# umr-lops/xsarsea

Hardware: AMD Instinct MI355X
Metric: Mpixels/s wind inversion (CMOD5.N, 20k x 20k sigma0) (higher is better)
Workload: dtype f64; 1 GPU; CMOD5.N mono-VV inversion (the metric's raster), 20000x20000 float32 sigma0/incidence + complex64 ancillary, default LUT 501x499x181 (90319 candidates/pixel), complex64 out, algo=pruned, sigma0 -> dB fused on the device; lines=20000, samples=20000, lines_rank0=20000, parallelism=row tiles x1

## Files before the change

xsarsea_amd/csrc/xsw_band.hpp:

```cpp
#pragma once
#include "xsw_device.hpp"

namespace xsw {

#ifndef XSW_BAND_MAX
#define XSW_BAND_MAX 64
#endif
#ifndef XSW_BAND_RAY_D
#define XSW_BAND_RAY_D 2
#endif
#ifndef XSW_LONG_RUN_MAX
#define XSW_LONG_RUN_MAX 128
#endif
#ifndef XSW_LONG_RUN_MAX_CUT
#define XSW_LONG_RUN_MAX_CUT 64
#endif
#ifndef XSW_SWEEP_MAX
#define XSW_SWEEP_MAX 128
#endif
#ifndef XSW_TAIL_SWEEP
#define XSW_TAIL_SWEEP 256
#endif
#ifndef XSW_B2_HARD_AREA
#define XSW_B2_HARD_AREA 256
#endif
#ifndef XSW_BAND_SEEDED
#define XSW_BAND_SEEDED 1
#endif
#ifndef XSW_BAND_RAYS
#define XSW_BAND_RAYS 3
#endif
#ifndef XSW_BAND_WG_WAVES
#define XSW_BAND_WG_WAVES 4
#endif
#ifndef XSW_BAND_WAVES
#define XSW_BAND_WAVES 8
#endif
#ifndef XSW_BAND_BATCH_S
#define XSW_BAND_BATCH_S 2
#endif
#ifndef XSW_BAND_BATCH
#define XSW_BAND_BATCH 4
#endif
#ifndef XSW_BAND_WAVES_CR
#define XSW_BAND_WAVES_CR 7
#endif
#ifndef XSW_BAND2_WAVES
#define XSW_BAND2_WAVES 4
#endif

struct BandSlot {
    double sn, thr_lo, thr_hi, ah, bh, m2;
    int inc_bin , rows , ipn ;
    int bin_hi ;
};

struct BandRec {
    double s, ah, bh;
    float d;
    int inc_tail;
    int rows;
    int ipn;
    unsigned idx;
    int flags;
};
struct Band2Slot;
constexpr int kBand2SlotBytes = 56;
template <typename T, typename TO, bool CR>
__device__ __forceinline__ void band2_core(const DevTables &L, const KArgs &A, const BandRec &r, bool in, bool searchable, int lane, Band2Slot *__restrict__ slots,
                                           int *__restrict__ res_, long long strip);

__device__ __forceinline__ unsigned long long ballot64(bool b) { return __builtin_amdgcn_ballot_w64(b); }

#ifndef XSW_BOUND_SLACK
#define XSW_BOUND_SLACK 4e-6f
#endif
#ifndef XSW_ARC_G
#define XSW_ARC_G 8
#endif
__device__ __forceinline__ unsigned window_arc(const unsigned short *__restrict__ inv_rows, const float *__restrict__ csphi32, int phi_pad, float wh0, float whs,
                                               bool on, int i_inc, int bin, int bhi, float uhx, float uhy, float jub, int ip_lo, int ncols, int w_lo, int w_hi)
{
    constexpr int G = XSW_ARC_G;
    static_assert(G == 4 || G == 8, "directions per table read");
    const int ii = on ? i_inc : 0;
    const unsigned short *__restrict__ inv_a = inv_rows + mul24_sv((unsigned)phi_pad, (unsigned)(ii * XSW_INV_BINS + (on ? bin : 0)));
    const unsigned short *__restrict__ inv_b = inv_rows + mul24_sv((unsigned)phi_pad, (unsigned)(ii * XSW_INV_BINS + (on ? min(bhi, XSW_INV_BINS - 1) : 0)));
    const bool capped = bhi < XSW_INV_BINS;
    const float m2 = uhx * uhx + uhy * uhy;
    int first = 0x7fff, last = -1;
    const int g0 = on ? (ip_lo & ~(G - 1)) : 0, ip_end = on ? ip_lo + ncols : 0;
    const int ngroups = wave_max_i(on ? (ip_end - g0 + G - 1) / G : 0);
#pragma unroll 1
    for (int k = 0; k < ngroups; ++k) {
        const int gp = g0 + k * G;
        const bool gact = on && gp < ip_end;
        const int gc = gact ? gp : 0;
        unsigned wa[G / 2], wb[G / 2];
        if constexpr (G == 8) {
            const uint4 qa = *(const uint4 *)(inv_a + gc), qb = *(const uint4 *)(inv_b + gc);
            wa[0] = qa.x; wa[1] = qa.y; wa[2] = qa.z; wa[3] = qa.w; wb[0] = qb.x; wb[1] = qb.y; wb[2] = qb.z; wb[3] = qb.w;
        } else {
            const uint2 qa = *(const uint2 *)(inv_a + gc), qb = *(const uint2 *)(inv_b + gc);
            wa[0] = qa.x; wa[1] = qa.y; wb[0] = qb.x; wb[1] = qb.y;
        }
#pragma unroll
        for (int h = 0; h < G / 2; ++h) {
            const float4 c4 = ((const float4 *)((const float2 *)csphi32 + gc))[h];
#pragma unroll
            for (int e = 0; e < 2; ++e) {
                const int ip = gc + 2 * h + e;
                const int ra = (int)((wa[h] >> (e * 16)) & 0xffffu), rb = (int)((wb[h] >> (e * 16)) & 0xffffu);
                const float uh = e ? uhx * c4.z + uhy * c4.w : uhx * c4.x + uhy * c4.y;
                const int lo = max(w_lo, ra), hi = capped ? min(w_hi, rb - 1) : w_hi;
                const float t = vminf(vmaxf(uh, fmaf((float)lo, whs, wh0)), fmaf((float)max(hi, lo), whs, wh0));
                const float jw = fmaf(t, t - 2.0f * uh, m2) - XSW_BOUND_SLACK * (m2 + t * (t + 2.0f * fabsf(uh)));
                const bool live = gact && ip >= ip_lo && ip < ip_end && lo <= hi && !(jw > jub);
                first = (live && first == 0x7fff) ? ip : first;
                last = live ? ip : last;
            }
        }
    }
    return last >= 0 ? (unsigned)first | ((unsigned)last << 16) : 0x00007fffu;
}
__device__ __forceinline__ double ld_co(const char *__restrict__ base, unsigned off0, int row, unsigned rowB)
{
    return *(const double *)(base + (off0 + __umul24((unsigned)row, rowB)));
}

#ifndef XSW_CHORD_MRG
#define XSW_CHORD_MRG 2e-3
#endif
template <int S, int K, bool COUNT>
__device__ __forceinline__ void co_band_pass(const DevTables &L, double inv_dsig, int lane,
                                             const BandSlot *slots , int *res ,
                                             int first, int count , unsigned &cand)
{
    constexpr int sweep_max = XSW_BAND_MAX;
    const double inf = __builtin_inf();
    const int q = lane / S, sl = lane & (S - 1);
    const bool valid = q < count;
    const int owner = valid ? first + q : lane;
    BandSlot B = slots[owner];
    if (!valid) { B.inc_bin = 0; B.rows = 0; B.ipn = 0; B.bin_hi = -1; }
    const int B_ip_lo = B.ipn & 0xffff, B_ncols = (int)((unsigned)B.ipn >> 16);
    const int w_lo = B.rows & 0xffff, w_hi = B.rows >> 16;
    const double thr_lo = B.thr_lo, thr_hi = B.thr_hi, sn = B.sn;
    const double wh0 = 0.5 * L.w0, whs = L.wstep_half;
    const char *__restrict__ base = (const char *)L.co;
    const unsigned rowB = (unsigned)L.phi_pad * 8u;
    const int i_inc = B.inc_bin & 0xffff;
    const unsigned slice0 = mul24_sv(rowB, mul24_sv((unsigned)L.n_w, (unsigned)i_inc));
    const unsigned short *__restrict__ inv_tab = L.inv_rows;
    const unsigned inv_rowB = (unsigned)L.phi_pad * 2u;
    const unsigned inv0 = mul24_sv(inv_rowB, (unsigned)(i_inc * XSW_INV_BINS) + ((unsigned)B.inc_bin >> 16));
    const unsigned inv1 = mul24_sv(inv_rowB, (unsigned)(i_inc * XSW_INV_BINS) + (unsigned)max(B.bin_hi, 0));
    double best = inf, second = inf;
    int brow = 0, bip = 0;
    unsigned ncand = 0;
    bool overflow = false;
    const int nchunks = S == 64 ? (__builtin_amdgcn_readfirstlane(B_ncols) + 64 * K - 1) / (64 * K) : 1;
#pragma unroll 1
    for (int ch = 0; ch < nchunks; ++ch) {
        bool act[K];
        int ip[K], r[K], nrow[K];
        unsigned off0[K];
        double U[K];
#pragma unroll
        for (int j = 0; j < K; ++j) {
            const int vcol = sl + S * j + S * K * ch;
            act[j] = valid && vcol < B_ncols;
            ip[j] = B_ip_lo + (act[j] ? vcol : 0);
            const unsigned ipB = (unsigned)ip[j] * 8u;
            const double2 cs = *(const double2 *)((const char *)L.csphi + 2u * ipB);
            U[j] = 2.0 * (B.ah * cs.x + B.bh * cs.y);
            off0[j] = slice0 + ipB;
        }
        int nmax = 0;
#pragma unroll
        for (int j = 0; j < K; ++j) {
            const unsigned o_first = inv0 + (unsigned)ip[j] * 2u, o_last = inv1 + (unsigned)ip[j] * 2u;
            const int ra = (int)*(const unsigned short *)((const char *)inv_tab + o_first);
            const int rb = (int)*(const unsigned short *)((const char *)inv_tab + o_last);
            r[j] = max(ra, w_lo);
            const int last = B.bin_hi >= 0 ? min(rb - 1, w_hi) : w_hi;
            nrow[j] = act[j] ? last - r[j] + 1 : 0;
            nmax = max(nmax, nrow[j]);
        }
#pragma unroll 1
        for (int t = 0; t < XSW_BAND_MAX; ++t) {
            unsigned long long left[K], any_left = 0ULL;
#pragma unroll
            for (int j = 0; j < K; ++j) { left[j] = ballot64(t < nrow[j]); any_left |= left[j]; }
            if (any_left == 0ULL) break;
#pragma unroll
            for (int j = 0; j < K; ++j) {
                if (left[j] == 0ULL) continue;
                const int rc = min(r[j] + t, w_hi);
                const double v = ld_co(base, off0[j], rc, rowB);
                const bool inb = t < nrow[j];
                const double wh = fma((double)rc, whs, wh0);
                const double dd = fma(v, inv_dsig, sn);
                double J = fma(dd, dd, wh * (wh - U[j]));
                J = __hiloint2double(inb ? __double2hiint(J) : 0x7FE00000, __double2loint(J));
                second = vmin(second, vmax(J, best));
                const bool lt = J < best;
                brow = lt ? rc : brow;
                if (K > 1 || S == 64) bip = lt ? ip[j] : bip;
                best = vmin(best, J);
                if (COUNT) ncand += inb ? 1u : 0u;
            }
        }
        const bool any = nmax > sweep_max;
        overflow = overflow || any;
        if (K == 1 && S != 64) bip = ip[0];
    }
    const int bflat = (int)__umul24((unsigned)brow, (unsigned)L.n_phi) + bip;
    const double gmin = S == 64 ? wave_min_d(best) : seg_min_d<S>(best);
    const double T = gmin + 1e-9 * (1.0 + fabs(gmin) + slots[owner].m2);
    const unsigned long long amb = ballot64(valid && (second <= T || overflow)), surv = ballot64(valid && best <= T);
    const unsigned long long segmask = S == 64 ? ~0ULL : (((1ULL << (S & 63)) - 1ULL) << ((q * S) & 63));
    const bool bad = (amb & segmask) != 0ULL || __popcll(surv & segmask) != 1 || !(gmin < 1e300);
    if (valid && ((!bad && best <= T) || (bad && sl == 0))) res[owner] = bad ? -1 : bflat;
    if (COUNT) {
        unsigned c = ncand;
        for (int off = 32; off > 0; off >>= 1) c += __shfl_xor(c, off);
        cand += c;
    }
}

__device__ __forceinline__ bool list_append(unsigned *__restrict__ count, unsigned *__restrict__ list, unsigned cap, bool flag, long long i, int lane)
{
    const unsigned long long um = __ballot(flag);
    if (!um) return false;
    unsigned base = 0;
    if (lane == 0) base = atomicAdd(count, (unsigned)__popcll(um));
    base = (unsigned)__builtin_amdgcn_readfirstlane((int)base);
    const unsigned at = base + __builtin_amdgcn_mbcnt_hi((unsigned)(um >> 32), __builtin_amdgcn_mbcnt_lo((unsigned)um, 0u));
    if (flag && at < cap) list[at] = (unsigned)i;
    return flag && at >= cap;
}
__device__ __forceinline__ void mask_mark(unsigned long long *__restrict__ mask, bool flag, long long i, long long strip, long long samples, int lane)
{
    const unsigned long long m = __ballot(flag);
    if (!m) return;
    if (strip >= 0) {
        if (lane == 0) atomicOr(&mask[strip], m);
    } else if (flag) {
        const long long ln = i / samples, sm = i - ln * samples;
        atomicOr(&mask[ln * ((samples + 63) >> 6) + (sm >> 6)], 1ULL << (sm & 63));
    }
}

template <typename T, typename TO, bool CR, bool COUNT>
__device__ __forceinline__ void wave_tail(const DevTables &L, const KArgs &A, long long i, bool in, int lane, int flags, int my_flat, long long strip,
                                          unsigned cand, int chain_slot = 0 )
{
    const bool to_b = A.list_b != nullptr && (flags & F_TO_B) != 0, to_c = (flags & F_TO_C) != 0;
    const double nan = __builtin_nan("");
    int my_icr = -1;
    const bool need_co = (flags & F_NEED_CO) != 0;
    bool unresolved = in && need_co && my_flat < 0;

    bool need_cr = false;
    if (CR && A.s_cr) {
        const double inc = ld<T>(A.inc, i);
        const T x = ((const T *)A.s_cr)[i];
        const double s_cr = to_db(x, A.is_db);
        const double dsig = A.dsig_cr ? (double)((const T *)A.dsig_cr)[i] : (double)(T)(x * (T)0 + (T)A.dsig_cr_scalar);
        need_cr = in && !(flags & (F_EARLY_NAN | F_CR_RAW_NAN)) && s_cr == s_cr && dsig == dsig;
        const bool here = need_cr && !unresolved;
        const int i_inc_cr = here ? nearest_index(L.inc_cr, L.n_inc_cr, inc, L.inc_cr_uniform != 0, L.inc_cr0, L.inv_inccrstep) : 0;
        const double aco = (here && need_co) ? L.abs_co[my_flat] : nan;
        bool undecided = here;
        const bool done = L.inv_cr ? search_cr_scan(L, here, i_inc_cr, s_cr, dsig, need_co, aco, my_icr, undecided)
                                   : search_cr_interval(L, here, i_inc_cr, s_cr, dsig, need_co, aco, my_icr, undecided);
        unresolved = unresolved || (need_cr && (undecided || !done));
        if (need_cr) flags |= F_NEED_CR;
    }
    if (COUNT && A.stats) {
        const unsigned long long done_co = __ballot(in && need_co && my_flat >= 0), done_cr = __ballot(need_cr && !unresolved);
        if (lane == 0) {
            atomicAdd(&A.stats[0], (unsigned long long)__popcll(done_co));
            atomicAdd(&A.stats[1], (unsigned long long)cand);
            if (chain_slot && A.stats_chain) atomicAdd(&A.stats[chain_slot], (unsigned long long)cand);
            atomicAdd(&A.stats[3], (unsigned long long)__popcll(done_cr));
        }
    }
    bool drop_b = false, drop_c = false;
    if (A.list_b) drop_b = A.rec_b ? (unresolved && to_b) : list_append(A.list_b_count, A.list_b, A.list_b_cap, unresolved && to_b, i, lane);
    if (A.list_c) drop_c = list_append(A.list_c_count, A.list_c, A.list_c_cap, unresolved && to_c && !to_b, i, lane);
    const bool for_c = A.list_c != nullptr && to_c && !to_b && !drop_c;
    const bool drop_g = list_append(A.list_count, A.list, A.list_cap, unresolved && !to_b && !for_c, i, lane);
    if (A.mask_g) {
        if (A.list_b) mask_mark(A.mask_b, drop_b, i, strip, A.samples, lane);
        mask_mark(A.mask_g, drop_g, i, strip, A.samples, lane);
    }
    if (in) {
        if (!unresolved) {
            Pixel Q;
            Q.flags = flags;
            Q.a_re = nan; Q.a_im = nan;
            if (A.anc) {
                typename Cx<T>::type z = ((const typename Cx<T>::type *)A.anc)[i];
                Q.a_re = (double)z.x;
                Q.a_im = (double)z.y;
            }
            store_pixel<TO, CR>(L, A, i, Q, my_flat, my_icr);
        }
    }
}

template <typename T, typename TO, bool CR, bool COUNT, int ROLE = 0>
__device__ __forceinline__ void band_wave(const DevTables &L, const KArgs &A, long long i, bool in, int lane, BandSlot *__restrict__ slots,
                                          int *__restrict__ res_, bool strip_walk = false ,
                                          long long strip = -1 )
{
    const double nan = __builtin_nan("");
    int flags, my_flat = -1, my_icr = -1;
    unsigned cand = 0;
    constexpr int NC = 11;
    int pos = -1, first[NC] = {}, ncls[NC] = {};
    bool skip = false;
    {
        Pixel P;
        load_pixel<T, false>(L, A, i, in, P);
        flags = P.flags;
        if (CR && A.s_cr) {
            const T x = ((const T *)A.s_cr)[i];
            const T dr = A.dsig_cr ? ((const T *)A.dsig_cr)[i] : (T)0;
            if (x != x || dr != dr) flags |= F_CR_RAW_NAN;
        }
        const unsigned long long todo = __ballot((P.flags & F_NEED_CO) != 0);
        bool eligb = false;
        int ncols_p = 0;
        if (todo) {
            bool loose = false;
            CoWindow W = co_window_lanes<XSW_BAND_RAYS, XSW_BAND_RAY_D, XSW_BAND_SEEDED != 0>(L, P, A.inv_dsig_co, fabs(A.dsig_co), loose);
            int w_hi_e = W.w_hi;
            bool has_tail = false;
            if (L.tail_min) {
                const bool fin1 = (P.flags & F_NEED_CO) != 0 && (P.flags & F_CO_FINITE) != 0;
                const int mono1 = L.mono_rows[fin1 ? P.i_inc : 0];
                if (fin1 && W.w_hi >= mono1 && W.ip_hi >= W.ip_lo) {
                    const int len = W.ip_hi - W.ip_lo + 1, k = min(31 - __clz(len), XSW_TAIL_LEVELS);
                    const double *tk = L.tail_min + mul24_sv((unsigned)L.phi_pad, (unsigned)(P.i_inc * (XSW_TAIL_LEVELS + 1) + k));
                    const double lo = fmin(tk[W.ip_lo], tk[k < XSW_TAIL_LEVELS ? W.ip_hi - (1 << k) + 1 : W.ip_lo]);
                    if (P.s_co + W.band_d < lo) w_hi_e = mono1 - 1;
                    else if (ROLE != 0 && mono1 >= 1 && W.w_hi - mono1 + 1 <= A.tail_max) { has_tail = true; w_hi_e = mono1 - 1; }
                }
            }
            const int nrows_p = w_hi_e - W.w_lo + 1;
            ncols_p = W.ip_hi - W.ip_lo + 1;
            const bool need = (P.flags & F_NEED_CO) != 0 && (P.flags & F_CO_FINITE) != 0 && ncols_p >= 1 && (nrows_p >= 1 || has_tail);
            if (ROLE == 2 && strip_walk) skip = !need || !(w_hi_e < L.mono_rows[need ? P.i_inc : 0]);
            eligb = need && w_hi_e < L.mono_rows[need ? P.i_inc : 0];
            if (ROLE != 2 && need && !eligb) flags |= F_TO_C;
            if (COUNT) cand += (unsigned)__popcll(__ballot(eligb)) * (unsigned)(2 * (32 - __clz((L.n_w + 1) >> 1)) + (XSW_BAND_RAYS - 1) * 2 * XSW_RAY_SIDE_STEPS);
            double thr_lo = P.s_co - W.band_d, thr_hi = P.s_co + W.band_d;
            int bin = 0, bhi = XSW_INV_BINS;
            if (eligb) {
                const double *g = L.inv_grid + 3 * P.i_inc;
                const double t0 = g[0], width = g[1];
                bin = (int)fmin(fmax((thr_lo - t0) * g[2], 0.0), (double)(XSW_INV_BINS - 1));
                if (bin > 0 && fma((double)bin, width, t0) > thr_lo) --bin;
                if (bin > 0 && fma((double)bin, width, t0) > thr_lo) bin = 0;
                bhi = (int)fmin(fmax((thr_hi - t0) * g[2], -1.0), (double)XSW_INV_BINS) + 1;
                if (bhi < XSW_INV_BINS && !(fma((double)bhi, width, t0) > thr_hi)) ++bhi;
                if (bhi < XSW_INV_BINS && !(fma((double)bhi, width, t0) > thr_hi)) bhi = XSW_INV_BINS;
            }
            if (ROLE != 0 && A.arc_min < 0x7fffffff) {
                const bool widep = eligb && !has_tail && ncols_p >= A.arc_min;
                if (__popcll(__ballot(widep)) >= A.arc_crowd) {
                    const double rs = W.band_d * fabs(A.inv_dsig_co);
                    const float jub32 = (float)(rs * rs) * (1.0f + 1e-5f) + 1e-5f;
                    double *park;
                    if constexpr (ROLE == 2) park = (double *)((char *)slots + lane * kBand2SlotBytes);
                    else park = (double *)&slots[lane];
                    park[0] = thr_lo; park[1] = thr_hi; park[2] = W.band_d; park[3] = P.s_co;
                    __asm__ volatile("" ::: "memory");
                    const unsigned arc = window_arc(L.inv_rows, (const float *)L.csphi32, L.phi_pad, (float)(0.5 * L.w0), (float)L.wstep_half, widep, P.i_inc, bin, bhi,
                                                    (float)(0.5 * P.a_re), (float)(0.5 * P.b_eff), jub32, W.ip_lo, ncols_p, W.w_lo, w_hi_e);
                    __asm__ volatile("" ::: "memory");
                    thr_lo = park[0]; thr_hi = park[1]; W.band_d = park[2]; P.s_co = park[3];
                    const int a_first = (int)(arc & 0xffffu), a_last = (int)(arc >> 16);
                    if (widep && a_last >= a_first) {
                        W.ip_lo = a_first;
                        ncols_p = a_last - a_first + 1;
                    }
                }
            }
            bool hard = false;
            int myc = NC;
            if (eligb) {
                const int nv = ncols_p;
                const int p2 = 31 - __clz(max(nv, 2) - 1);
                myc = nv <= 4 ? 0 : min(2 * p2 - 3 + (nv > (3 << (p2 - 1)) ? 1 : 0), NC - 1);
            }
            if (ROLE == 1 || (ROLE == 2 && strip_walk)) {
                int run = 0;
                if (eligb) {
                    const unsigned tab0 = (unsigned)(P.i_inc * XSW_INV_BINS);
                    auto run_at = [&](int ip) {
                        const int ra = (int)L.inv_rows[mul24_sv((unsigned)L.phi_pad, tab0 + (unsigned)bin) + (unsigned)ip];
                        const int rb = bhi < XSW_INV_BINS ? (int)L.inv_rows[mul24_sv((unsigned)L.phi_pad, tab0 + (unsigned)bhi) + (unsigned)ip] : w_hi_e + 1;
                        return min(rb - 1, w_hi_e) - max(ra, W.w_lo) + 1;
                    };
                    run = run_at(P.ipr);
                    if (has_tail) run = max(run, 0) + (W.w_hi - w_hi_e);
                }
                const bool long_one = eligb && run > ((w_hi_e < W.w_hi && !has_tail) ? XSW_LONG_RUN_MAX_CUT : XSW_LONG_RUN_MAX);
                const bool big_area = eligb && !long_one && run * ncols_p > A.area_max;
                const bool crowded = __popcll(__ballot(big_area)) >= A.b2_crowd;
                if (big_area && crowded && run * ncols_p <= A.area_crowd_max) flags |= F_B2_CROWD;
                if (long_one || (big_area && (flags & F_B2_CROWD) == 0)) {
                    myc = NC;
                    eligb = false;
                    if (ROLE == 2) skip = true;
                    if (ROLE == 1) flags |= F_TO_C;
                }
                hard = has_tail || run * ncols_p >= XSW_B2_HARD_AREA || ncols_p >= 64;
                const bool handed = eligb && (run >= A.long_run || has_tail || ncols_p >= A.wide_min);
                if (ROLE == 1 && handed) {
                    myc = NC;
                    eligb = false;
                    flags |= F_TO_B;
                }
                if (ROLE == 2 && eligb && !handed) {
                    myc = NC;
                    eligb = false;
                    skip = true;
                }
            }
            int base = 0;
#pragma unroll
            for (int c = 0; c < NC; ++c) {
                const unsigned long long m = __ballot(myc == c);
                const int rank = (int)__builtin_amdgcn_mbcnt_hi((unsigned)(m >> 32), __builtin_amdgcn_mbcnt_lo((unsigned)m, 0u));
                pos = myc == c ? base + rank : pos;
                first[c] = base;
                ncls[c] = __popcll(m);
                base += ncls[c];
            }
#pragma unroll
            for (int c = 0; c + 1 < NC; ++c) {
                const int np = 64 / (2 << (c >> 1)), npn = 64 / (2 << ((c + 1) >> 1));
                const int rem = ncls[c] % np;
                const int added = (ncls[c + 1] + rem + npn - 1) / npn - (ncls[c + 1] + npn - 1) / npn;
                if (rem > 0 && added == 0) { ncls[c] -= rem; ncls[c + 1] += rem; first[c + 1] -= rem; }
            }
#pragma unroll
            for (int c = 0; c < NC; ++c) {
                first[c] = __builtin_amdgcn_readfirstlane(first[c]);
                ncls[c] = __builtin_amdgcn_readfirstlane(ncls[c]);
            }
            const bool to_rec = ROLE == 1 && A.rec_b != nullptr && (flags & F_TO_B) != 0;
            if constexpr (ROLE == 2) {
                const bool mine = in && !(strip_walk && (skip || (flags & F_NEED_CO) == 0));
                BandRec r;
                r.s = P.s_co; r.ah = 0.5 * P.a_re; r.bh = 0.5 * P.b_eff; r.d = __double2float_ru(W.band_d);
                r.inc_tail = P.i_inc | ((has_tail ? W.w_hi - w_hi_e : 0) << 16);
                r.rows = W.w_lo | (w_hi_e << 16); r.ipn = W.ip_lo | (ncols_p << 16);
                r.idx = (unsigned)i; r.flags = flags | F_B2_HARD;
                band2_core<T, TO, CR>(L, A, r, mine, mine && eligb, lane, (Band2Slot *)slots, res_, strip);
                return;
            }
            BandSlot b;
            if (eligb) {
                const double ah = 0.5 * P.a_re, bh = 0.5 * P.b_eff;
                b.sn = -P.s_co * A.inv_dsig_co; b.thr_lo = thr_lo; b.thr_hi = thr_hi;
                b.ah = ah; b.bh = bh; b.m2 = ah * ah + bh * bh;
                b.inc_bin = P.i_inc | (bin << 16); b.rows = W.w_lo | (w_hi_e << 16); b.ipn = W.ip_lo | (ncols_p << 16);
                b.bin_hi = bhi < XSW_INV_BINS ? bhi : -1;
            }
            if (ROLE == 1 && A.rec_b != nullptr) {
                const unsigned long long hm = __ballot(to_rec);
                if (hm) {
                    unsigned at0 = 0;
                    if (lane == 0) at0 = atomicAdd(A.list_b_count, (unsigned)__popcll(hm));
                    at0 = (unsigned)__builtin_amdgcn_readfirstlane((int)at0);
                    const unsigned at = at0 + __builtin_amdgcn_mbcnt_hi((unsigned)(hm >> 32), __builtin_amdgcn_mbcnt_lo((unsigned)hm, 0u));
                    if (to_rec && at < A.list_b_cap) {
                        BandRec r;
                        r.s = P.s_co; r.ah = 0.5 * P.a_re; r.bh = 0.5 * P.b_eff; r.d = __double2float_ru(W.band_d);
                        r.inc_tail = P.i_inc | ((has_tail ? W.w_hi - w_hi_e : 0) << 16);
                        r.rows = W.w_lo | (w_hi_e << 16); r.ipn = W.ip_lo | (ncols_p << 16);
                        r.idx = (unsigned)i;
                        r.flags = (flags & ~F_TO_B) | (hard ? F_B2_HARD : 0);
                        ((BandRec *)A.rec_b)[at] = r;
                        flags |= F_REC_DONE;
                    }
                }
            }
            if (eligb) {
                slots[pos] = b;
#ifdef XSW_TIMING_STAGE1_ONLY
                res_[pos] = 0;
#else
                res_[pos] = -1;
#endif
            }
        }
    }
    res_[64 + lane] = pos;
    __builtin_amdgcn_fence(__ATOMIC_RELEASE, "wavefront");
    __builtin_amdgcn_wave_barrier();
    __builtin_amdgcn_fence(__ATOMIC_ACQUIRE, "wavefront");
#ifndef XSW_TIMING_STAGE1_ONLY
    {
        auto run = [&](auto seg, auto kk, int c) {
            constexpr int S = decltype(seg)::value, K = decltype(kk)::value;
            for (int p = 0; p < ncls[c]; p += 64 / S)
                co_band_pass<S, K, COUNT>(L, A.inv_dsig_co, lane, slots, res_, first[c] + p, min(64 / S, ncls[c] - p), cand);
        };
        using two = std::integral_constant<int, 2>;
        using three = std::integral_constant<int, 3>;
#ifndef XSW_BAND_WIDE_K
#define XSW_BAND_WIDE_K three
#endif
        run(std::integral_constant<int, 2>{}, two{}, 0);
        run(std::integral_constant<int, 2>{}, three{}, 1);
        run(std::integral_constant<int, 4>{}, two{}, 2);
        run(std::integral_constant<int, 4>{}, three{}, 3);
        run(std::integral_constant<int, 8>{}, two{}, 4);
        run(std::integral_constant<int, 8>{}, three{}, 5);
        run(std::integral_constant<int, 16>{}, two{}, 6);
        run(std::integral_constant<int, 16>{}, three{}, 7);
        run(std::integral_constant<int, 32>{}, two{}, 8);
        run(std::integral_constant<int, 32>{}, three{}, 9);
        run(std::integral_constant<int, 64>{}, XSW_BAND_WIDE_K{}, 10);
    }
#endif
    __builtin_amdgcn_fence(__ATOMIC_RELEASE, "wavefront");
    __builtin_amdgcn_wave_barrier();
    __builtin_amdgcn_fence(__ATOMIC_ACQUIRE, "wavefront");
    pos = res_[64 + lane];
    if (pos >= 0) my_flat = res_[pos];
    if (ROLE == 1 && (flags & F_REC_DONE) != 0) in = false;
    if (ROLE == 2 && strip_walk) {
        skip = skip || (flags & F_NEED_CO) == 0;
        in = in && !skip;
    }
    wave_tail<T, TO, CR, COUNT>(L, A, i, in, lane, flags, my_flat, strip, cand);
}

template <typename T, typename TO, bool CR, bool COUNT, int ROLE = 0>
__global__ __launch_bounds__(64 * XSW_BAND_WG_WAVES, CR ? XSW_BAND_WAVES_CR : XSW_BAND_WAVES) void k_invert_band(DevTables L, KArgs A)
{
    const int lane = threadIdx.x & 63, wv = threadIdx.x >> 6;
    __shared__ BandSlot slots[XSW_BAND_WG_WAVES][64];
    __shared__ int res_[XSW_BAND_WG_WAVES][128];
    const long long strips_per_line = (A.samples + 63) >> 6;
    const long long cols_per_xcd = (strips_per_line + 7) >> 3;
    const long long xcd = blockIdx.x & 7;
    const long long col = xcd * cols_per_xcd + blockIdx.y;
    const long long line = (long long)(blockIdx.x >> 3) * XSW_BAND_WG_WAVES + wv;
    if (col >= strips_per_line || line >= A.lines) return;
    const long long smp = col * 64 + lane;
    const bool in = smp < A.samples;
    const long long i = line * A.samples + (in ? smp : A.samples - 1);
    band_wave<T, TO, CR, COUNT, ROLE>(L, A, i, in, lane, slots[wv], res_[wv], false, line * strips_per_line + col);
}

}
```

xsarsea_amd/csrc/xsw_invert_tu.hip:

```cpp
#include <hip/hip_runtime.h>

#include <algorithm>
#include <cstdlib>
#include <string>

#include "xsw_host.hpp"
#include "xsw_band.hpp"
#include "xsw_band2.hpp"
#include "xsw_blocks.hpp"
#include "xsw_exhaustive.hpp"

using namespace xsw;

#ifndef XSW_B2_AREA
#define XSW_B2_AREA 2048
#endif
#ifndef XSW_LONG_RUN_DEFAULT
#define XSW_LONG_RUN_DEFAULT 5
#endif
#ifndef XSW_ARC_MIN
#define XSW_ARC_MIN 32
#endif
#ifndef XSW_ARC_CROWD
#define XSW_ARC_CROWD 48
#endif
#ifndef XSW_B2_CROWD
#define XSW_B2_CROWD 24
#endif
#ifndef XSW_B2_WIDE
#define XSW_B2_WIDE 0
#endif
#ifndef XSW_B2_REFINE_MIN
#define XSW_B2_REFINE_MIN 16
#endif
#ifndef XSW_BLOCK_MIN
#define XSW_BLOCK_MIN 1024
#endif

template <typename T, typename TO>
static int launch_invert(xsw_ctx *c, const KArgs &A_in, int algo, const LaunchCtl &lc, std::string &err)
{
    KArgs A = A_in;
    const long long strips_per_line = (A.samples + 63) / 64, line_groups = (A.lines + 3) / 4;
    const long long nblocks = 8 * ((strips_per_line + 7) / 8) * line_groups;
    if (nblocks > 0x7fffffffLL) return seterr(err, XSW_EINVAL, "raster too large for one launch");
    const bool mono = !A.s_cr && !A.out_cr && !A.code_cr;
    if (algo == XSW_ALGO_EXHAUSTIVE || algo == XSW_ALGO_EXHAUSTIVE_F64)
        return launch_exhaustive<T, TO>(c->T, A, lc.stream, algo == XSW_ALGO_EXHAUSTIVE) == hipSuccess
                   ? XSW_OK : seterr(err, XSW_EHIP, "exhaustive launch failed: %s", hipGetErrorString(hipGetLastError()));
    static const int block_min_env = getenv("XSW_BLOCK_MIN") ? std::max(0, atoi(getenv("XSW_BLOCK_MIN"))) : XSW_BLOCK_MIN;
    A.block_min = block_min_env;
    static const bool band_off = getenv("XSW_NO_BAND") != nullptr;
    if (algo == XSW_ALGO_PRUNED && !band_off && lc.list && A.s_co && c->T.prunable && c->T.mono_rows && c->T.inv_rows && c->T.co_off32 && c->T.band_mul24 &&
        (!A.s_cr || c->T.cr_monotone) && A.n < (1LL << 32)) {
        KArgs B = A;
        B.list_count = lc.list;
        B.list = lc.list + 16;
        B.list_cap = (unsigned)std::min<size_t>(lc.list_cap, 0xfffffff0u);
        static const int long_run_env = getenv("XSW_LONG_RUN") ? std::max(0, atoi(getenv("XSW_LONG_RUN"))) : XSW_LONG_RUN_DEFAULT;
        const bool count_inst = A.stats && !A.stats_chain;
        const bool band2 = long_run_env > 0 && !count_inst;
        if (band2) { B.list_b_count = lc.list + 1; B.list_b = lc.list + 16 + lc.list_cap; B.list_b_cap = (unsigned)std::min<size_t>(XSW_LIST_B_SHARE * lc.list_cap, 0xfffffff0u); }
        static const bool records_off = getenv("XSW_NO_RECORDS") != nullptr;
        static_assert(sizeof(BandRec) == XSW_REC_BYTES, "XSW_REC_BYTES (xsw_host.hpp) is sizeof(BandRec)");
        B.rec_b = (band2 && !records_off) ? lc.rec_b : nullptr;
        static const bool blocks_kernel_off = getenv("XSW_NO_BLOCKS_KERNEL") != nullptr;
        const bool blocks3 = c->T.blk != nullptr && c->T.blk_span_ok && !blocks_kernel_off && c->T.n_w < 32768 && c->T.n_phi < 32768;
        if (blocks3) { B.list_c_count = lc.list + 2; B.list_c = lc.list + 16 + (1 + XSW_LIST_B_SHARE) * lc.list_cap; B.list_c_cap = (unsigned)std::min<size_t>(XSW_LIST_C_SHARE * lc.list_cap, 0xfffffff0u); }
        B.long_run = long_run_env;
        static const int area_max_env = getenv("XSW_B2_AREA") ? std::max(1, atoi(getenv("XSW_B2_AREA"))) : XSW_B2_AREA;
        B.area_max = c->T.blk ? area_max_env : 0x7fffffff;
        static const int crowd_env = getenv("XSW_B2_CROWD") ? std::max(1, atoi(getenv("XSW_B2_CROWD"))) : XSW_B2_CROWD;
        B.b2_crowd = crowd_env;
        B.area_crowd_max = 1 << 20;
        static const int wide_env = getenv("XSW_B2_WIDE") ? std::max(0, atoi(getenv("XSW_B2_WIDE"))) : XSW_B2_WIDE;
        B.wide_min = wide_env > 0 ? wide_env : 0x7fffffff;
        static const int arc_min_env = getenv("XSW_ARC_MIN") ? atoi(getenv("XSW_ARC_MIN")) : XSW_ARC_MIN;
        static const int arc_crowd_env = getenv("XSW_ARC_CROWD") ? std::max(1, atoi(getenv("XSW_ARC_CROWD"))) : XSW_ARC_CROWD;
        B.arc_min = (arc_min_env > 0 && c->T.csphi32) ? arc_min_env : 0x7fffffff;
        B.arc_crowd = arc_crowd_env;
        static const int refine_min_env = getenv("XSW_B2_REFINE_MIN") ? std::max(0, atoi(getenv("XSW_B2_REFINE_MIN"))) : XSW_B2_REFINE_MIN;
        B.b2_refine_min = refine_min_env;
        static const int b2_rows_env = getenv("XSW_B2_ROWS_MAX") ? std::max(1, atoi(getenv("XSW_B2_ROWS_MAX"))) : XSW_B2_ROWS_MAX;
        B.b2_rows_max = b2_rows_env;
        static const int tail_max_env = getenv("XSW_TAIL_SWEEP") ? std::min(std::max(0, atoi(getenv("XSW_TAIL_SWEEP"))), 30000) : XSW_TAIL_SWEEP;
        B.tail_max = (band2 && c->T.tail_min) ? tail_max_env : 0;
        static const bool masks_off = getenv("XSW_NO_STRIP_MASKS") != nullptr;
        const size_t nstrips = (size_t)(strips_per_line * A.lines);
        if (lc.masks && nstrips <= lc.mask_strips && !masks_off) {
            B.mask_g = lc.masks; B.mask_b = lc.masks + nstrips;
            if (hipMemsetAsync(lc.masks, 0, 2 * nstrips * sizeof(unsigned long long), lc.stream) != hipSuccess) return seterr(err, XSW_EHIP, "strip-mask reset failed");
        }
        if (hipMemsetAsync(lc.list, 0, 3 * sizeof(unsigned), lc.stream) != hipSuccess) return seterr(err, XSW_EHIP, "work-list reset failed");
        const unsigned list_blocks = (unsigned)std::min<long long>(nblocks, 256 * 8);
        const long long cols_per_xcd = (strips_per_line + 7) / 8;
        const long long band_groups = (A.lines + XSW_BAND_WG_WAVES - 1) / XSW_BAND_WG_WAVES;
        if (8 * band_groups > 0x7fffffffLL || cols_per_xcd > 65535) return seterr(err, XSW_EINVAL, "raster too large for one launch");
        const dim3 band_grid((unsigned)(8 * band_groups), (unsigned)cols_per_xcd), band_block(64 * XSW_BAND_WG_WAVES);
        if (lc.timing) timing_mark(c);
        if (count_inst) {
            if (mono) hipLaunchKernelGGL((k_invert_band<T, TO, false, true>), band_grid, band_block, 0, lc.stream, c->T, B);
            else hipLaunchKernelGGL((k_invert_band<T, TO, true, true>), band_grid, band_block, 0, lc.stream, c->T, B);
        } else if (band2) {
            if (mono) hipLaunchKernelGGL((k_invert_band<T, TO, false, false, 1>), band_grid, band_block, 0, lc.stream, c->T, B);
            else hipLaunchKernelGGL((k_invert_band<T, TO, true, false, 1>), band_grid, band_block, 0, lc.stream, c->T, B);
        } else if (mono) {
            hipLaunchKernelGGL((k_invert_band<T, TO, false, false>), band_grid, band_block, 0, lc.stream, c->T, B);
        } else {
            hipLaunchKernelGGL((k_invert_band<T, TO, true, false>), band_grid, band_block, 0, lc.stream, c->T, B);
        }
        if (lc.timing) timing_mark(c);
        if (band2) {
            const dim3 b2_grid((unsigned)std::min<long long>(nblocks, 256 * XSW_BAND2_WAVES));
            if (mono) hipLaunchKernelGGL((k_invert_band2<T, TO, false>), b2_grid, band_block, 0, lc.stream, c->T, B);
            else hipLaunchKernelGGL((k_invert_band2<T, TO, true>), b2_grid, band_block, 0, lc.stream, c->T, B);
        }
        if (lc.timing) timing_mark(c);
        if (blocks3) {
            const dim3 bl_grid((unsigned)std::min<long long>(nblocks, 256 * XSW_BLOCKS_WAVES));
            if (mono) hipLaunchKernelGGL((k_invert_blocks<T, TO, false>), bl_grid, dim3(256), 0, lc.stream, c->T, B);
            else hipLaunchKernelGGL((k_invert_blocks<T, TO, true>), bl_grid, dim3(256), 0, lc.stream, c->T, B);
        }
        if (lc.timing) timing_mark(c);
        if (mono) hipLaunchKernelGGL((k_invert_list<T, TO, false>), dim3(list_blocks), dim3(256), 0, lc.stream, c->T, B);
        else hipLaunchKernelGGL((k_invert_list<T, TO, true>), dim3(list_blocks), dim3(256), 0, lc.stream, c->T, B);
        if (lc.timing) timing_mark(c);
        const hipError_t e = hipGetLastError();
        if (e != hipSuccess) return seterr(err, XSW_EHIP, "launch failed: %s", hipGetErrorString(e));
        return XSW_OK;
    }
    if (algo == XSW_ALGO_PRUNED && mono)
        hipLaunchKernelGGL((k_invert<T, TO, 1, false>), dim3((unsigned)nblocks), dim3(256), 0, lc.stream, c->T, A);
    else if (algo == XSW_ALGO_PRUNED)
        hipLaunchKernelGGL((k_invert<T, TO, 1>), dim3((unsigned)nblocks), dim3(256), 0, lc.stream, c->T, A);
    else
        hipLaunchKernelGGL((k_invert<T, TO, 3>), dim3((unsigned)nblocks), dim3(256), 0, lc.stream, c->T, A);
    const hipError_t e = hipGetLastError();
    if (e != hipSuccess) return seterr(err, XSW_EHIP, "launch failed: %s", hipGetErrorString(e));
    return XSW_OK;
}


#ifndef XSW_PAIR
#error "compile with -DXSW_PAIR=0..3"
#endif
#if XSW_PAIR == 0
int xsw_launch_invert_ff(xsw_ctx *c, const KArgs &A, int algo, const LaunchCtl &lc, std::string &err) { return launch_invert<float, float>(c, A, algo, lc, err); }
#elif XSW_PAIR == 1
int xsw_launch_invert_fd(xsw_ctx *c, const KArgs &A, int algo, const LaunchCtl &lc, std::string &err) { return launch_invert<float, double>(c, A, algo, lc, err); }
#elif XSW_PAIR == 2
int xsw_launch_invert_df(xsw_ctx *c, const KArgs &A, int algo, const LaunchCtl &lc, std::string &err) { return launch_invert<double, float>(c, A, algo, lc, err); }
#else
int xsw_launch_invert_dd(xsw_ctx *c, const KArgs &A, int algo, const LaunchCtl &lc, std::string &err) { return launch_invert<double, double>(c, A, algo, lc, err); }
#endif
```

Measured before the change: 10590 Mpixels/s.

## Pool band-pass class queues across waves of a workgroup

Each wave's per-class candidate counts are published to shared memory, merged into workgroup-wide class queues through an index map, and the resulting passes are dealt round-robin to the waves. Partially filled passes from individual waves are meant to be merged so fewer mostly idle band passes run. In exchange it adds two workgroup barriers, an indirection through the shared map, and keeps dead waves alive so they can take part in the barriers. It also adds optional pass-count stats behind an ifdef.

```diff
diff --git a/xsarsea_amd/csrc/xsw_band.hpp b/xsarsea_amd/csrc/xsw_band.hpp
--- a/xsarsea_amd/csrc/xsw_band.hpp
+++ b/xsarsea_amd/csrc/xsw_band.hpp
@@ -33,6 +33,10 @@
 #ifndef XSW_BAND_WG_WAVES
 #define XSW_BAND_WG_WAVES 4
 #endif
+#ifndef XSW_BAND_POOL
+#define XSW_BAND_POOL 1
+#endif
+static_assert(XSW_BAND_WG_WAVES % 4 == 0 || !XSW_BAND_POOL, "pooled class counts are read as four bytes per word");
 #ifndef XSW_BAND_WAVES
 #define XSW_BAND_WAVES 8
 #endif
@@ -54,6 +58,17 @@
     int inc_bin , rows , ipn ;
     int bin_hi ;
 };
+
+constexpr int kBandClasses = 11;
+struct BandPool {
+    alignas(4) unsigned char cnt[kBandClasses][XSW_BAND_WG_WAVES];
+    unsigned short map[64 * XSW_BAND_WG_WAVES];
+};
+__device__ __forceinline__ int byte_sum4(unsigned x)
+{
+    x = (x & 0x00ff00ffu) + ((x >> 8) & 0x00ff00ffu);
+    return (int)((x & 0xffffu) + (x >> 16));
+}
 
 struct BandRec {
     double s, ah, bh;
@@ -134,13 +149,14 @@
 template <int S, int K, bool COUNT>
 __device__ __forceinline__ void co_band_pass(const DevTables &L, double inv_dsig, int lane,
                                              const BandSlot *slots , int *res ,
-                                             int first, int count , unsigned &cand)
+                                             int first, int count , unsigned &cand,
+                                             const unsigned short *map = nullptr )
 {
     constexpr int sweep_max = XSW_BAND_MAX;
     const double inf = __builtin_inf();
     const int q = lane / S, sl = lane & (S - 1);
     const bool valid = q < count;
-    const int owner = valid ? first + q : lane;
+    const int owner = valid ? (map ? (int)map[first + q] : first + q) : lane;
     BandSlot B = slots[owner];
     if (!valid) { B.inc_bin = 0; B.rows = 0; B.ipn = 0; B.bin_hi = -1; }
     const int B_ip_lo = B.ipn & 0xffff, B_ncols = (int)((unsigned)B.ipn >> 16);
@@ -314,13 +330,30 @@
 template <typename T, typename TO, bool CR, bool COUNT, int ROLE = 0>
 __device__ __forceinline__ void band_wave(const DevTables &L, const KArgs &A, long long i, bool in, int lane, BandSlot *__restrict__ slots,
                                           int *__restrict__ res_, bool strip_walk = false ,
-                                          long long strip = -1 )
+                                          long long strip = -1 ,
+                                          BandPool *__restrict__ pool = nullptr )
 {
     const double nan = __builtin_nan("");
     int flags, my_flat = -1, my_icr = -1;
     unsigned cand = 0;
-    constexpr int NC = 11;
-    int pos = -1, first[NC] = {}, ncls[NC] = {};
+    constexpr int NC = kBandClasses;
+    constexpr bool POOLED = XSW_BAND_POOL && ROLE != 2;
+    constexpr int WG = XSW_BAND_WG_WAVES, PK = POOLED ? 64 * WG : 64;
+    int pos = -1, myc = NC, first[NC] = {}, ncls[NC] = {};
+    auto settle_queues = [&]() {
+#pragma unroll
+        for (int c = 0; c + 1 < NC; ++c) {
+            const int np = 64 / (2 << (c >> 1)), npn = 64 / (2 << ((c + 1) >> 1));
+            const int rem = ncls[c] % np;
+            const int added = (ncls[c + 1] + rem + npn - 1) / npn - (ncls[c + 1] + npn - 1) / npn;
+            if (rem > 0 && added == 0) { ncls[c] -= rem; ncls[c + 1] += rem; first[c + 1] -= rem; }
+        }
+#pragma unroll
+        for (int c = 0; c < NC; ++c) {
+            first[c] = __builtin_amdgcn_readfirstlane(first[c]);
+            ncls[c] = __builtin_amdgcn_readfirstlane(ncls[c]);
+        }
+    };
     bool skip = false;
     {
         Pixel P;
@@ -391,7 +424,7 @@
                 }
             }
             bool hard = false;
-            int myc = NC;
+            myc = NC;
             if (eligb) {
                 const int nv = ncols_p;
                 const int p2 = 31 - __clz(max(nv, 2) - 1);
@@ -442,18 +475,7 @@
                 ncls[c] = __popcll(m);
                 base += ncls[c];
             }
-#pragma unroll
-            for (int c = 0; c + 1 < NC; ++c) {
-                const int np = 64 / (2 << (c >> 1)), npn = 64 / (2 << ((c + 1) >> 1));
-                const int rem = ncls[c] % np;
-                const int added = (ncls[c + 1] + rem + npn - 1) / npn - (ncls[c + 1] + npn - 1) / npn;
-                if (rem > 0 && added == 0) { ncls[c] -= rem; ncls[c + 1] += rem; first[c + 1] -= rem; }
-            }
-#pragma unroll
-            for (int c = 0; c < NC; ++c) {
-                first[c] = __builtin_amdgcn_readfirstlane(first[c]);
-                ncls[c] = __builtin_amdgcn_readfirstlane(ncls[c]);
-            }
+            if constexpr (!POOLED) settle_queues();
             const bool to_rec = ROLE == 1 && A.rec_b != nullptr && (flags & F_TO_B) != 0;
             if constexpr (ROLE == 2) {
                 const bool mine = in && !(strip_walk && (skip || (flags & F_NEED_CO) == 0));
@@ -502,16 +524,65 @@
             }
         }
     }
-    res_[64 + lane] = pos;
-    __builtin_amdgcn_fence(__ATOMIC_RELEASE, "wavefront");
-    __builtin_amdgcn_wave_barrier();
-    __builtin_amdgcn_fence(__ATOMIC_ACQUIRE, "wavefront");
+    res_[PK + lane] = pos;
+    const int wv = POOLED ? __builtin_amdgcn_readfirstlane((int)(threadIdx.x >> 6)) : 0;
+    if constexpr (POOLED) {
+        static_assert((WG & (WG - 1)) == 0, "passes are dealt to the waves modulo XSW_BAND_WG_WAVES");
+        if (lane == 0) {
+#pragma unroll
+            for (int c = 0; c < NC; ++c) pool->cnt[c][wv] = (unsigned char)ncls[c];
+        }
+        __syncthreads();
+        int e = 0, base = 0;
+#pragma unroll
+        for (int c = 0; c < NC; ++c) {
+            int n = 0, before = 0;
+#pragma unroll
+            for (int k = 0; k < WG / 4; ++k) {
+                const unsigned x = (unsigned)__builtin_amdgcn_readfirstlane((int)((const unsigned *)pool->cnt[c])[k]);
+                const int lo = wv - 4 * k;
+                n += byte_sum4(x);
+                before += byte_sum4(lo >= 4 ? x : lo <= 0 ? 0u : x & ((1u << (8 * lo)) - 1u));
+            }
+            e = myc == c ? base + before - first[c] : e;
+            first[c] = base;
+            ncls[c] = n;
+            base += n;
+        }
+        settle_queues();
+        if (pos >= 0) pool->map[pos + e] = (unsigned short)(wv * 64 + pos);
+        __syncthreads();
+    } else {
+        __builtin_amdgcn_fence(__ATOMIC_RELEASE, "wavefront");
+        __builtin_amdgcn_wave_barrier();
+        __builtin_amdgcn_fence(__ATOMIC_ACQUIRE, "wavefront");
+    }
+#ifdef XSW_BAND_PASS_STATS
+    unsigned long long pst[8] = {};
+#endif
 #ifndef XSW_TIMING_STAGE1_ONLY
     {
+        int dealt = 0;
         auto run = [&](auto seg, auto kk, int c) {
-            constexpr int S = decltype(seg)::value, K = decltype(kk)::value;
-            for (int p = 0; p < ncls[c]; p += 64 / S)
-                co_band_pass<S, K, COUNT>(L, A.inv_dsig_co, lane, slots, res_, first[c] + p, min(64 / S, ncls[c] - p), cand);
+            constexpr int S = decltype(seg)::value, K = decltype(kk)::value, np = 64 / S;
+            if constexpr (POOLED) {
+                const int npass = (ncls[c] + np - 1) / np;
+                for (int p = (wv - dealt) & (WG - 1); p < npass; p += WG) {
+                    co_band_pass<S, K, COUNT>(L, A.inv_dsig_co, lane, slots - 64 * wv, res_ - 64 * wv, first[c] + p * np, min(np, ncls[c] - p * np), cand,
+                                              pool->map);
+#ifdef XSW_BAND_PASS_STATS
+                    pst[c < 7 ? c : 7] += (1ULL << 32) + (unsigned long long)min(np, ncls[c] - p * np);
+#endif
+                }
+                dealt += npass;
+            } else {
+                for (int p = 0; p < ncls[c]; p += np) {
+                    co_band_pass<S, K, COUNT>(L, A.inv_dsig_co, lane, slots, res_, first[c] + p, min(np, ncls[c] - p), cand);
+#ifdef XSW_BAND_PASS_STATS
+                    pst[c < 7 ? c : 7] += (1ULL << 32) + (unsigned long long)min(np, ncls[c] - p);
+#endif
+                }
+            }
         };
         using two = std::integral_constant<int, 2>;
         using three = std::integral_constant<int, 3>;
@@ -531,10 +602,21 @@
         run(std::integral_constant<int, 64>{}, XSW_BAND_WIDE_K{}, 10);
     }
 #endif
-    __builtin_amdgcn_fence(__ATOMIC_RELEASE, "wavefront");
-    __builtin_amdgcn_wave_barrier();
-    __builtin_amdgcn_fence(__ATOMIC_ACQUIRE, "wavefront");
-    pos = res_[64 + lane];
+    if constexpr (POOLED) {
+        __syncthreads();
+    } else {
+        __builtin_amdgcn_fence(__ATOMIC_RELEASE, "wavefront");
+        __builtin_amdgcn_wave_barrier();
+        __builtin_amdgcn_fence(__ATOMIC_ACQUIRE, "wavefront");
+    }
+#ifdef XSW_BAND_PASS_STATS
+    if (A.stats && lane == 0) {
+#pragma unroll
+        for (int k = 0; k < 8; ++k)
+            if (pst[k]) atomicAdd(&A.stats[k], pst[k]);
+    }
+#endif
+    pos = res_[PK + lane];
     if (pos >= 0) my_flat = res_[pos];
     if (ROLE == 1 && (flags & F_REC_DONE) != 0) in = false;
     if (ROLE == 2 && strip_walk) {
@@ -550,16 +632,27 @@
     const int lane = threadIdx.x & 63, wv = threadIdx.x >> 6;
     __shared__ BandSlot slots[XSW_BAND_WG_WAVES][64];
     __shared__ int res_[XSW_BAND_WG_WAVES][128];
+#if XSW_BAND_POOL
+    __shared__ BandPool pool;
+#endif
     const long long strips_per_line = (A.samples + 63) >> 6;
     const long long cols_per_xcd = (strips_per_line + 7) >> 3;
     const long long xcd = blockIdx.x & 7;
     const long long col = xcd * cols_per_xcd + blockIdx.y;
     const long long line = (long long)(blockIdx.x >> 3) * XSW_BAND_WG_WAVES + wv;
+    const long long smp = col * 64 + lane;
+#if XSW_BAND_POOL
+    if (col >= strips_per_line) return;
+    const bool live = line < A.lines;
+    const bool in = live && smp < A.samples;
+    const long long i = (live ? line : A.lines - 1) * A.samples + (smp < A.samples ? smp : A.samples - 1);
+    band_wave<T, TO, CR, COUNT, ROLE>(L, A, i, in, lane, slots[wv], &res_[0][0] + 64 * wv, false, line * strips_per_line + col, &pool);
+#else
     if (col >= strips_per_line || line >= A.lines) return;
-    const long long smp = col * 64 + lane;
     const bool in = smp < A.samples;
     const long long i = line * A.samples + (in ? smp : A.samples - 1);
     band_wave<T, TO, CR, COUNT, ROLE>(L, A, i, in, lane, slots[wv], res_[wv], false, line * strips_per_line + col);
-}
-
-}
+#endif
+}
+
+}
diff --git a/xsarsea_amd/csrc/xsw_invert_tu.hip b/xsarsea_amd/csrc/xsw_invert_tu.hip
--- a/xsarsea_amd/csrc/xsw_invert_tu.hip
+++ b/xsarsea_amd/csrc/xsw_invert_tu.hip
@@ -110,6 +110,9 @@
             hipLaunchKernelGGL((k_invert_band<T, TO, true, false>), band_grid, band_block, 0, lc.stream, c->T, B);
         }
         if (lc.timing) timing_mark(c);
+#ifdef XSW_BAND_PASS_STATS
+        B.stats = nullptr;
+#endif
         if (band2) {
             const dim3 b2_grid((unsigned)std::min<long long>(nblocks, 256 * XSW_BAND2_WAVES));
             if (mono) hipLaunchKernelGGL((k_invert_band2<T, TO, false>), b2_grid, band_block, 0, lc.stream, c->T, B);
```

Measured after the change: 10890 Mpixels/s, median of 6. +2.8%, better.
